# maruchitatsuki/python-based-Sequential-Monte-Carlo-method-with-likelihood-tempering

Hardware: AMD Instinct MI355X
Metric: particle-mutation-steps/sec (higher is better)
Workload: dtype f64

## Files before the change

include/smc_hip.h:

```cpp
#ifndef SMC_HIP_H
#define SMC_HIP_H

#include <stddef.h>
#include <stdint.h>

#ifdef __cplusplus
extern "C" {
#endif

#define SMC_ABI_VERSION 3
#define SMC_MAX_DIM 8
#define SMC_MAX_ESS_CAND 16
#define SMC_MAX_RANKS 64

#define SMC_SET_PRED 0
#define SMC_SET_FILT 1

#define SMC_PRIOR_UNIFORM 0
#define SMC_PRIOR_NORMAL 1
#define SMC_PRIOR_FLAT 2

#define SMC_PRIOR_MODE_MASK 0
#define SMC_PRIOR_MODE_RATIO_MASK 1
#define SMC_PRIOR_MODE_RATIO 2
// ... 125 lines not shown
                             size_t max_staging_bytes, double *mean, double *sd, double *lower, double *upper, int64_t *n_finite,
                             int64_t *n_failed, int64_t *attempts, double *kernel_ms);
int smc_user_pointwise(smc_ctx *ctx, const double *particle, int64_t n, double *ll, int64_t *n_failed, int64_t *attempts);
int smc_user_pointwise_summary(smc_ctx *ctx, int set, size_t max_staging_bytes, int64_t *n, double *max, double *sum_exp, double *mean,
                               double *m2, double *pit, int64_t *n_failed, int64_t *attempts, double *kernel_ms);
int smc_user_sweep_counters(smc_ctx *ctx, int64_t out[4]);
int smc_meth_sweep_counters(smc_ctx *ctx, int64_t out[4]);
int smc_meth_sweep_check(smc_ctx *ctx, int64_t out[5]);
int smc_meth_download_solves(smc_ctx *ctx, double *flows, int32_t *status, int64_t n);
int smc_set_prior(smc_ctx *ctx, const int *kind, const double *a, const double *b, int dim);
int smc_set_prior_mode(smc_ctx *ctx, int mode);

#define SMC_RESAMPLE_RESIDUAL_SYSTEMATIC 0
#define SMC_RESAMPLE_SYSTEMATIC 1
#define SMC_RESAMPLE_MULTINOMIAL 2
int smc_set_early_reject(smc_ctx *ctx, int enable);
int smc_set_stiff_first(smc_ctx *ctx, int enable);
int smc_set_cost_order(smc_ctx *ctx, int enable);
int smc_set_fast_tail(smc_ctx *ctx, int enable);
int smc_set_share_replicates(smc_ctx *ctx, int enable);
int smc_mm_group_replicates(const double *t, const double *S0, int n_ex, int n_t, int *primary, int *partner);
int smc_mm_share_info(smc_ctx *ctx, int *n_solve, int64_t *shared_attempts);
int smc_set_start_reject(smc_ctx *ctx, int enable);
int smc_mm_start_reject_info(smc_ctx *ctx, int64_t *not_started);
double smc_mm_reject_threshold(double lk1, double gamma, double rr, double sigma, int n_ex, int n_t, double pratio, int in_support);
int smc_set_in_phase(smc_ctx *ctx, int enable);
int smc_set_exact_pow(smc_ctx *ctx, int enable);
int smc_set_resampling(smc_ctx *ctx, int scheme);

int smc_upload_particles(smc_ctx *ctx, int set, const double *aos, int64_t n);
int smc_download_particles(smc_ctx *ctx, int set, double *aos, int64_t n);
int smc_upload_lk(smc_ctx *ctx, int set, const double *lk, int64_t n);
int smc_download_lk(smc_ctx *ctx, int set, double *lk, int64_t n);
int smc_download_accept_flags(smc_ctx *ctx, uint8_t *flags, int64_t n);
int smc_download_item_info(smc_ctx *ctx, int32_t *info, int64_t n);
int smc_download_item_sums(smc_ctx *ctx, double *sums, int64_t n);
int smc_commit_filt_to_pred(smc_ctx *ctx);
int smc_sample_prior_device(smc_ctx *ctx, uint64_t seed, int64_t global_offset);

int smc_loglik(smc_ctx *ctx, int set, int64_t *n_failed, int64_t *rk_attempts);
int smc_mm_loglik_host(smc_ctx *ctx, const double *particle, int64_t n, double *lk, double *pred, int64_t *n_failed,
                       int64_t *rk_attempts);

int smc_max_lk_local(smc_ctx *ctx, double *max_lk);
int smc_ess_partials(smc_ctx *ctx, double max_lk, const double *gm, int n_cand, double *sum_w, double *sum_w2);
int smc_max_lk_global(smc_ctx *ctx, double *max_lk);
// ... 93 lines not shown
```

python-based-sequential-monte-carlo-method-with-likelihood-tempering_amd/binding.py:

```python
from __future__ import annotations

import ctypes
import os
import re

_HERE = os.path.dirname(os.path.abspath(__file__))
LIB_PATH = os.environ.get("SMC_HIP_LIB") or os.path.join(_HERE, "libsmc_hip.so")
HEADER_PATH = os.path.join(os.path.dirname(_HERE), "include", "smc_hip.h")

SMC_SET_PRED, SMC_SET_FILT = 0, 1
SMC_USER_METHOD_RK45, SMC_USER_METHOD_BDF = 0, 1
SMC_USER_MAX_OBS = 8
SMC_USER_MAX_INPUTS, SMC_USER_MAX_KNOTS = 8, 4096
SMC_USER_MAX_EVENTS, SMC_USER_MAX_EVENT_VALUES = 256, 8
SMC_USER_MAX_ROOTS, SMC_USER_MAX_ROOT_FIRES = 4, 256
USER_METHODS = {"RK45": SMC_USER_METHOD_RK45, "BDF": SMC_USER_METHOD_BDF}
SMC_PRIOR_UNIFORM, SMC_PRIOR_NORMAL, SMC_PRIOR_FLAT = 0, 1, 2
SMC_PRIOR_MODE_MASK, SMC_PRIOR_MODE_RATIO_MASK, SMC_PRIOR_MODE_RATIO = 0, 1, 2
PRIOR_MODES = {"mask": 0, "ratio_mask": 1, "ratio": 2}
RESAMPLING = {"residual_systematic": 0, "systematic": 1, "multinomial": 2}
SMC_MAX_ESS_CAND = 16
SMC_PRED_MAX_PROBS = 16
SMC_ABI_VERSION = 3
SMC_SWEEP_COUNTER_WORDS = 14
# ... 88 lines not shown
    "smc_user_model_dump_source7": (cint, [ctypes.c_char_p, cint, cint, cint, cint, cint, cint, cint, cint, cint, cint, cint,
                                            ctypes.c_char_p]),
    "smc_user_predict": (cint, [c_ctx, c_dp, i64, c_dp, c_dp, c_i64p, c_i64p]),
    "smc_user_predict_at": (cint, [c_ctx, c_dp, i64, c_dp, c_dp, cint, cint, c_dp, c_i64p, c_i64p]),
    "smc_user_predict_summary": (cint, [c_ctx, cint, c_dp, c_dp, cint, cint, c_dp, cint, cint, u64, i64, ctypes.c_size_t, c_dp, c_dp,
                                         c_dp, c_dp, c_i64p, c_i64p, c_i64p, c_dp]),
    "smc_user_pointwise": (cint, [c_ctx, c_dp, i64, c_dp, c_i64p, c_i64p]),
    "smc_user_pointwise_summary": (cint, [c_ctx, cint, ctypes.c_size_t, c_i64p, c_dp, c_dp, c_dp, c_dp, c_dp, c_i64p, c_i64p, c_dp]),
    "smc_user_sweep_counters": (cint, [c_ctx, c_i64p]),
    "smc_meth_sweep_counters": (cint, [c_ctx, c_i64p]),
    "smc_meth_sweep_check": (cint, [c_ctx, c_i64p]),
    "smc_meth_download_solves": (cint, [c_ctx, c_dp, ctypes.POINTER(ctypes.c_int32), i64]),
    "smc_set_prior": (cint, [c_ctx, c_ip, c_dp, c_dp, cint]),
    "smc_set_prior_mode": (cint, [c_ctx, cint]),
    "smc_set_resampling": (cint, [c_ctx, cint]),
    "smc_set_early_reject": (cint, [c_ctx, cint]),
    "smc_set_stiff_first": (cint, [c_ctx, cint]),
    "smc_set_cost_order": (cint, [c_ctx, cint]),
    "smc_set_fast_tail": (cint, [c_ctx, cint]),
    "smc_set_share_replicates": (cint, [c_ctx, cint]),
    "smc_mm_group_replicates": (cint, [c_dp, c_dp, cint, cint, c_ip, c_ip]),
    "smc_mm_share_info": (cint, [c_ctx, c_ip, c_i64p]),
    "smc_set_start_reject": (cint, [c_ctx, cint]),
    "smc_mm_start_reject_info": (cint, [c_ctx, c_i64p]),
    "smc_mm_reject_threshold": (ctypes.c_double, [ctypes.c_double, ctypes.c_double, ctypes.c_double, ctypes.c_double, cint, cint,
                                                  ctypes.c_double, cint]),
    "smc_set_in_phase": (cint, [c_ctx, cint]),
    "smc_set_exact_pow": (cint, [c_ctx, cint]),
    "smc_exchange_plan": (cint, [cint, cint, i64, c_i64p, c_i64p, c_i64p, c_i64p, c_i64p, c_i64p, c_i64p, c_i64p, c_i64p, c_i64p]),
    "smc_upload_particles": (cint, [c_ctx, cint, c_dp, i64]),
    "smc_download_particles": (cint, [c_ctx, cint, c_dp, i64]),
    "smc_upload_lk": (cint, [c_ctx, cint, c_dp, i64]),
    "smc_download_lk": (cint, [c_ctx, cint, c_dp, i64]),
    "smc_download_accept_flags": (cint, [c_ctx, c_u8p, i64]),
    "smc_download_item_info": (cint, [c_ctx, ctypes.POINTER(ctypes.c_int32), i64]),
    "smc_download_item_sums": (cint, [c_ctx, c_dp, i64]),
    "smc_debug_set_order": (cint, [c_ctx, ctypes.POINTER(ctypes.c_int32), i64, cint]),
    "smc_commit_filt_to_pred": (cint, [c_ctx]),
    "smc_sample_prior_device": (cint, [c_ctx, u64, i64]),
    "smc_loglik": (cint, [c_ctx, cint, c_i64p, c_i64p]),
    "smc_mm_loglik_host": (cint, [c_ctx, c_dp, i64, c_dp, c_dp, c_i64p, c_i64p]),
    "smc_max_lk_local": (cint, [c_ctx, c_dp]),
    "smc_ess_partials": (cint, [c_ctx, f64, c_dp, cint, c_dp, c_dp]),
    "smc_max_lk_global": (cint, [c_ctx, c_dp]),
    "smc_ess_partials_global": (cint, [c_ctx, f64, c_dp, cint, c_dp, c_dp]),
    "smc_ess_search_global": (cint, [c_ctx, c_dp, cint, cint, c_dp, c_dp, c_dp]),
# ... 87 lines not shown
```

python-based-sequential-monte-carlo-method-with-likelihood-tempering_amd/csrc/mm_kernels.hip:

```cpp
#include <hip/hip_runtime.h>

#include <cstdlib>

#include "mh_control.h"
#include "mm_rk45.h"
#include "solve_sched.h"
#include "philox.h"
#include "prior.h"
#include "smc_internal.h"
#include "reject_bound.h"

namespace smc {

constexpr int kInfoAttemptsMask = 0x1fffffff, kInfoCancelled = 1 << 29, kInfoFailed = 1 << 30;
constexpr double kSumCancelled = -1.0;

#ifndef SMC_STIFF_RATIO
#define SMC_STIFF_RATIO 60.0
#endif
constexpr double kStiffRatio = SMC_STIFF_RATIO;
#ifndef SMC_SOLO_RATIO
#define SMC_SOLO_RATIO 1000.0
#endif
constexpr double kSoloRatio = SMC_SOLO_RATIO;
static_assert(kSoloRatio >= kStiffRatio, "the index-ordered pass skips what either list holds by the stiff predicate alone");
__device__ __forceinline__ bool mm_is_stiff(double Vmax, double Km) { return Km > 0.0 && Vmax > kStiffRatio * Km; }
__device__ __forceinline__ bool mm_is_solo(double Vmax, double Km) { return Km > 0.0 && Vmax > kSoloRatio * Km; }
__device__ __forceinline__ void stiff_list_append(const StiffList &sl, int64_t p, double Vmax, double Km) {
    if (mm_is_solo(Vmax, Km)) {
        const unsigned k = atomicAdd(sl.count + 1, 1u);
        if (k < sl.solo_cap) {
            sl.particles[sl.cap - 1 - (int64_t)k] = (int32_t)p;
            return;
        }
    }
    sl.particles[atomicAdd(sl.count, 1u)] = (int32_t)p;
}
constexpr int kCostBuckets = 128, kCostBlocks = 256;
// ... 251 lines not shown
constexpr int kStartLookFrom = SMC_START_LOOK_FROM;
static_assert(kStartLookFrom >= 1, "group 0 is handed out first: it has no finished sibling");

struct SolveArgs {
    const double *theta;
    int64_t stride, n;
    const uint8_t *p0;
    double *sum_r2;
    int *info;
    double *pred;
    unsigned long long *queue;
    const RejectArgs *rej;
    const int32_t *stiff_list;
    const unsigned *stiff_count;
    int64_t stiff_cap;
    unsigned solo_cap;
    int patience;
    int start_look;
    const int32_t *order;
    const unsigned *n_ordered;
    const SortedProposal *sorted;
    const MHControl *ctl;
};

struct ShareArgs {
    const int *groups;
    int n_solve;
};

#ifdef SMC_NO_OWN_SGPR
template <class T> __device__ __forceinline__ T own_sgpr(T v) { return v; }
#else
__device__ __forceinline__ double own_sgpr(double v) {
    double r;
    asm volatile("s_mov_b64 %0, %1" : "=s"(r) : "s"(v));
    return r;
}
template <class T>
__device__ __forceinline__ T *own_sgpr(T *p) {
    T *r;
    asm volatile("s_mov_b64 %0, %1" : "=s"(r) : "s"(p));
    return r;
}
__device__ __forceinline__ int own_sgpr(int v) {
    int r;
    asm volatile("s_mov_b32 %0, %1" : "=s"(r) : "s"(v));
    return r;
}
#endif

__device__ __forceinline__ double mm_loglik_term(double c0, double sum_r2, double s2) { return c0 - sum_r2 / (2.0 * s2); }

__device__ __forceinline__ void publish_item(double *sums, int *infos, int64_t idx, double sum_r2, int info) {
    __hip_atomic_store(reinterpret_cast<unsigned long long *>(sums) + idx, (unsigned long long)__double_as_longlong(sum_r2),
                       __ATOMIC_RELAXED, __HIP_MEMORY_SCOPE_AGENT);
    infos[idx] = info;
}
__device__ __forceinline__ void publish_item(const SolveArgs &a, int64_t idx, double sum_r2, int info) {
    publish_item(a.sum_r2, a.info, idx, sum_r2, info);
}

__device__ __forceinline__ bool mm_certainly_rejected(const MMModel &mm, const SolveArgs &a, int64_t p, int e_self,
                                                      double partial_self, int e_partner = -1, double partial_partner = 0.0) {
    const double sigma = mm.est_sigma ? a.theta[2 * a.stride + p] : mm.sigma_fixed;
    if (!(sigma > 0.0)) return false;
    const double s2 = sigma * sigma;
    const double c0 = (-0.5 * mm.n_t) * log(2.0 * 3.141592653589793 * s2);
    double lk2_bound = 0.0;
    for (int k = 0; k < mm.n_ex; ++k) {
        double S = 0.0;
        if (k == e_self) {
            S = partial_self;
        } else if (k == e_partner) {
            S = partial_partner;
        } else {
            const double v = sibling_sum(a.sum_r2, (int64_t)k * a.n + p);
            if (v < 0.0) return true;
            if (v == v) S = v;
        }
        lk2_bound += mm_loglik_term(c0, S, s2);
    }
    return reject_bound_fails(*a.rej, p, lk2_bound);
}

template <bool WRITE_PRED, bool EXACT, bool FAST, bool SHARE = false>
struct MMOps {
    struct Item {
        MMItem s;
        int64_t out_idx;
        double *pred;
    };
    static constexpr int kPoolWords = smc::kPoolWords;
    const MMModel &mm;
    const SolveArgs &a;
    const double2 *s_tp;
    const double *s_S0;
    long long n;
    int n_ex, n_t;
    const int32_t *list;
    unsigned n_list;
    const int32_t *solo;
    unsigned n_solo;
    double rtol, atol;
    int patience;
    long long n_pos;
    double *pub_sums;
    int *pub_info;
    double *s_sum2;
    const int *s_grp;
    int look;

    __device__ __forceinline__ double *sum2_word() const { return SHARE ? s_sum2 + threadIdx.x : nullptr; }
    __device__ __forceinline__ int partner_distance(const Item &it) const { return SHARE ? it.s.t_off >> kSharePartnerShift : 0; }
    __device__ __forceinline__ double partner_sum(const Item &it) const { return it.s.i_out == 0 ? 0.0 : *sum2_word(); }

    __device__ __forceinline__ int start(long long p, int e, bool from_list, Item &nb) const {
        const bool masked = !a.n_ordered && a.p0 && a.p0[p] == 0;
        return start_values(p, e, from_list, masked, a.theta[p], a.theta[a.stride + p], mm.est_sigma ? a.theta[2 * a.stride + p] : mm.sigma_fixed, nb);
    }
    __device__ __forceinline__ int start_values(long long p, int e, bool from_list, bool masked, double Vmax, double Km, double sigma,
                                                Item &nb) const {
        int d_e = 0;
        const int g_self = e;
        if (SHARE) {
            const int g = e;
            e = s_grp[2 * g];
            const int partner = s_grp[2 * g + 1];
            d_e = partner < 0 ? 0 : partner - e;
        }
        const int n_ex_data = SHARE ? mm.n_ex : n_ex;
        const int64_t out_idx2 = (int64_t)(e + d_e) * a.n + p;
        nb.out_idx = (int64_t)e * a.n + p;
        nb.pred = nullptr;
        if (!from_list && list && !masked && mm_is_stiff(Vmax, Km)) return kStartSkipped;
        if (look != 0 && !from_list && !masked && g_self >= kStartLookFrom) {
            double fin = 0.0;
            bool dead = false;
            const unsigned long long *sums = reinterpret_cast<const unsigned long long *>(pub_sums) + p;
            for (int k = SHARE ? mm.n_ex : n_ex; k > 0; --k, sums += n) {
                const double v = __longlong_as_double((long long)__hip_atomic_load(sums, __ATOMIC_RELAXED, __HIP_MEMORY_SCOPE_AGENT));
                dead = dead || v < 0.0;
                fin += v >= 0.0 ? v : 0.0;
            }
            const double T = *reinterpret_cast<const double *>(sums);
            if (dead || (fin >= T && fin <= 1.7976931348623157e308)) {
                publish_item(a, nb.out_idx, kSumCancelled, 0 | kInfoCancelled);
                if (SHARE && d_e != 0) publish_item(a, out_idx2, kSumCancelled, 0 | kInfoCancelled);
                return kStartDone;
            }
        }
        if (masked || sigma <= 0.0) {
            publish_item(a, nb.out_idx, 0.0, 0);
            if (SHARE && d_e != 0) publish_item(a, out_idx2, 0.0, 0);
            if (WRITE_PRED) {
                double *pp = a.pred + ((size_t)p * n_ex_data + e) * n_t;
                for (int i = 0; i < n_t; ++i) pp[i] = quiet_nan();
                if (SHARE && d_e != 0)
                    for (int i = 0; i < n_t; ++i) pp[d_e * n_t + i] = quiet_nan();
// ... 97 lines not shown
    __device__ __forceinline__ Item broadcast(const Item &it, int src) const {
        Item u;
        u.s.negVmax = lane_value(it.s.negVmax, src);
        u.s.Km = lane_value(it.s.Km, src);
        u.s.S0 = lane_value(it.s.S0, src);
        u.s.t = lane_value(it.s.t, src);
        u.s.y = lane_value(it.s.y, src);
        u.s.f = lane_value(it.s.f, src);
        u.s.h_abs = lane_value(it.s.h_abs, src);
        u.s.min_step = lane_value(it.s.min_step, src);
        u.s.t_bound = lane_value(it.s.t_bound, src);
        u.s.t_next = lane_value(it.s.t_next, src);
        u.s.sum_r2 = lane_value(it.s.sum_r2, src);
        u.s.t_off = __builtin_amdgcn_readlane(it.s.t_off, src);
        u.s.i_out = __builtin_amdgcn_readlane(it.s.i_out, src);
        u.s.attempts = __builtin_amdgcn_readlane(it.s.attempts, src);
        u.s.rejected = __builtin_amdgcn_readlane((int)it.s.rejected, src) != 0;
        u.out_idx = lane_value_ll(it.out_idx, src);
        u.pred = WRITE_PRED ? (double *)lane_value_ll((long long)it.pred, src) : nullptr;
        if (SHARE) *sum2_word() = lane_value(*sum2_word(), src);
        return u;
    }
    __device__ __forceinline__ bool reject_enabled() const { return a.rej != nullptr; }
    __device__ __forceinline__ bool certainly_rejected(const Item &it) const {
        const int e_self = (int)(it.out_idx / a.n);
        if (SHARE) {
            const int d_e = partner_distance(it);
            return mm_certainly_rejected(mm, a, it.out_idx - (int64_t)e_self * a.n, e_self, it.s.sum_r2, d_e != 0 ? e_self + d_e : -1,
                                         partner_sum(it));
        }
        return mm_certainly_rejected(mm, a, it.out_idx - (int64_t)e_self * a.n, e_self, it.s.sum_r2);
    }
    __device__ __forceinline__ void cancel(Item &it) const {
        publish_item(a, it.out_idx, kSumCancelled, it.s.attempts | kInfoCancelled);
        if (SHARE) {
            const int d_e = partner_distance(it);
            if (d_e != 0) publish_item(a, it.out_idx + (int64_t)d_e * a.n, kSumCancelled, it.s.attempts | kInfoCancelled);
        }
    }
};

template <bool WRITE_PRED, bool EXACT, bool FAST, bool SHARE = false>
__device__ __forceinline__ void mm_solve_body(const MMModel &mm, const SolveArgs &a, const ShareArgs *sh = nullptr) {
    extern __shared__ double2 smem_tp[];
    if (a.ctl && __builtin_amdgcn_readfirstlane(a.ctl->stop)) return;
    const int n_ex = mm.n_ex, n_t = mm.n_t;
    double2 *s_tp = smem_tp;
    double *s_S0 = reinterpret_cast<double *>(s_tp + (SHARE ? 2 : 1) * n_ex * (n_t + 1));
    if (SHARE)
        mm_table_fill_shared(s_tp, mm.t, mm.P_obs, n_ex, n_t, threadIdx.x, blockDim.x, sh->groups, sh->n_solve);
    else
        mm_table_fill(s_tp, mm.t, mm.P_obs, n_ex, n_t, threadIdx.x, blockDim.x);
    if (threadIdx.x < n_ex) s_S0[threadIdx.x] = mm.S0[threadIdx.x];
    double *s_sum2 = s_S0 + ((n_ex + 1) & ~1) + (size_t)(kSolveBlock / kWave) * (kPoolWords * kWave);
// ... 363 lines not shown
                         bool start_look = false) {
    const bool share = share_on(ctx);
    MMModel mm = ctx->mm;
    mm.partner_mask = 0;
    SolveArgs a{};
    a.theta = theta;
    a.stride = stride;
    a.n = n;
    a.p0 = p0;
    a.sum_r2 = ctx->d_sum_r2;
    a.info = ctx->d_info;
    a.pred = pred;
    a.queue = ctx->d_queue;
    a.rej = reject ? ctx->d_reject : nullptr;
    a.stiff_list = sl.particles;
    a.stiff_count = sl.count;
    a.stiff_cap = sl.cap;
    a.solo_cap = sl.solo_cap;
    a.patience = patience;
    a.order = order;
    a.n_ordered = cost_ordered ? cost_n_ordered(ctx) : nullptr;
    a.sorted = static_cast<const SortedProposal *>(ctx->d_sorted);
    a.ctl = ctl;
    a.start_look = reject && start_look;
#ifdef SMC_DEBUG_PATIENCE_ENV
    if (const char *e = getenv("SMC_DEBUG_PATIENCE")) a.patience = atoi(e);
#endif
    if (!queue_cleared) (void)hipMemsetAsync(ctx->d_queue, 0, sizeof(unsigned long long), ctx->stream);
    const size_t lds = solve_lds_bytes(mm.n_ex, mm.n_t, share);
    const bool exact = ctx->exact_pow != 0;
    const bool fast = use_fast_tail(ctx, n);
    void (*kern)(MMModel, SolveArgs) =
        pred ? (exact ? mm_solve_kernel<true, true, false> : fast ? mm_solve_kernel<true, false, true> : mm_solve_kernel<true, false, false>)
             : (exact ? mm_solve_kernel<false, true, false> : fast ? mm_solve_kernel<false, false, true> : mm_solve_kernel<false, false, false>);
    void (*kern_share)(MMModel, SolveArgs, ShareArgs) =
        pred ? (exact ? mm_solve_share_kernel<true, true, false> : fast ? mm_solve_share_kernel<true, false, true> : mm_solve_share_kernel<true, false, false>)
             : (exact ? mm_solve_share_kernel<false, true, false> : fast ? mm_solve_share_kernel<false, false, true> : mm_solve_share_kernel<false, false, false>);
    if (lds > 48 * 1024 && !ctx->solve_lds_raised) {
        hipError_t e = hipSuccess;
        for (const void *f : {reinterpret_cast<const void *>(&mm_solve_kernel<true, true, false>), reinterpret_cast<const void *>(&mm_solve_kernel<true, false, false>),
                              reinterpret_cast<const void *>(&mm_solve_kernel<true, false, true>), reinterpret_cast<const void *>(&mm_solve_kernel<false, true, false>),
                              reinterpret_cast<const void *>(&mm_solve_kernel<false, false, false>), reinterpret_cast<const void *>(&mm_solve_kernel<false, false, true>),
                              reinterpret_cast<const void *>(&mm_solve_share_kernel<true, true, false>), reinterpret_cast<const void *>(&mm_solve_share_kernel<true, false, false>),
                              reinterpret_cast<const void *>(&mm_solve_share_kernel<true, false, true>), reinterpret_cast<const void *>(&mm_solve_share_kernel<false, true, false>),
                              reinterpret_cast<const void *>(&mm_solve_share_kernel<false, false, false>), reinterpret_cast<const void *>(&mm_solve_share_kernel<false, false, true>)})
            if (e == hipSuccess) e = hipFuncSetAttribute(f, hipFuncAttributeMaxDynamicSharedMemorySize, 128 * 1024);
        if (e != hipSuccess) {
// ... 86 lines not shown
```

python-based-sequential-monte-carlo-method-with-likelihood-tempering_amd/csrc/smc_api.hip:

```cpp
#include <hip/hip_runtime.h>
#include <rccl/rccl.h>

#include <cmath>
#include <cstddef>
#include <cstdio>
#include <cstdlib>
#include <chrono>
#include <condition_variable>
#include <cstring>
#include <mutex>
#include <new>

#include "exchange_plan.h"
#include "replicate_groups.h"
#include "smc_internal.h"
#include "stage_kernels.h"

using namespace smc;

static thread_local std::string g_err;

#define HIPC(ctx, call)                                                                                   \
    do {                                                                                                  \
        hipError_t e_ = (call);                                                                           \
// ... 133 lines not shown
const char *smc_last_error(const smc_ctx *ctx) { return ctx ? ctx->err.c_str() : g_err.c_str(); }

int smc_create(smc_ctx **out, int device, int64_t n_local, int64_t n_global, int dim) {
    if (!out) return fail(nullptr, "smc_create: out is NULL");
    *out = nullptr;
    if (n_local <= 0 || n_global < n_local) return fail(nullptr, "smc_create: need 0 < n_local <= n_global");
    if (n_global >= (int64_t)1 << 31) return fail(nullptr, "smc_create: n_global must be < 2^31");
    if (dim < 1 || dim > SMC_MAX_DIM) return fail(nullptr, "smc_create: dim out of range");
    int ndev = 0;
    HIPC((smc_ctx *)nullptr, hipGetDeviceCount(&ndev));
    if (device < 0 || device >= ndev) return fail(nullptr, "smc_create: no such HIP device");
    HIPC((smc_ctx *)nullptr, hipSetDevice(device));
    smc_ctx *c = new (std::nothrow) smc_ctx();
    if (!c) return fail(nullptr, "smc_create: out of host memory");
    c->device = device;
    c->dim = dim;
    c->n_local = n_local;
    c->n_global = n_global;
    {
        const char *e = getenv("SMC_SHARE_REPLICATES");
        c->share_env_off = e ? atoi(e) == 0 : false;
        e = getenv("SMC_START_REJECT");
        c->start_reject_env_off = e ? atoi(e) == 0 : false;
    }
#define CK(call)                                   \
    do {                                           \
        hipError_t e_ = (call);                    \
        if (e_ != hipSuccess) {                    \
            g_err = std::string(#call) + ": " + hipGetErrorString(e_); \
            smc_destroy(c);                        \
            return 1;                              \
        }                                          \
    } while (0)
    CK(hipStreamCreateWithFlags(&c->stream, hipStreamNonBlocking));
    const size_t nb = (size_t)n_local * sizeof(double);
    for (int s = 0; s < 2; ++s) {
        CK(hipMalloc(&c->set[s].theta, nb * dim));
        CK(hipMalloc(&c->set[s].lk, nb));
        CK(hipMemsetAsync(c->set[s].theta, 0, nb * dim, c->stream));
        CK(hipMemsetAsync(c->set[s].lk, 0, nb, c->stream));
        c->set[s].stride = n_local;
    }
    CK(hipMalloc(&c->r_ac, (size_t)n_local));
    CK(hipMemsetAsync(c->r_ac, 0, (size_t)n_local, c->stream));
    CK(hipMalloc(&c->d_counters, sizeof(SweepCounters)));
    CK(hipMalloc(&c->d_queue, 2 * sizeof(unsigned long long)));
// ... 331 lines not shown
    c->order_debug_patience = patience;
    return 0;
}
int smc_set_cost_order(smc_ctx *c, int enable) {
    if (!c) return fail(nullptr, "NULL context");
    c->cost_order = enable != 0;
    return 0;
}
int smc_set_fast_tail(smc_ctx *c, int enable) {
    if (!c) return smc_fail(nullptr, "NULL context");
    c->fast_tail = enable != 0;
    return 0;
}
int smc_set_share_replicates(smc_ctx *c, int enable) {
    if (!c) return fail(nullptr, "NULL context");
    c->share_replicates = enable != 0;
    return 0;
}
int smc_set_start_reject(smc_ctx *c, int enable) {
    if (!c) return fail(nullptr, "NULL context");
    c->start_reject = enable != 0;
    return 0;
}
int smc_mm_start_reject_info(smc_ctx *c, int64_t *not_started) {
    if (!c) return fail(nullptr, "NULL context");
    if (not_started) *not_started = c->w_not_started;
    return 0;
}
double smc_mm_reject_threshold(double lk1, double gamma, double rr, double sigma, int n_ex, int n_t, double pratio, int in_support) {
    return mm_reject_threshold(lk1, gamma, rr, sigma, n_ex, n_t, pratio, in_support);
}
int smc_mm_group_replicates(const double *t, const double *S0, int n_ex, int n_t, int *primary, int *partner) {
    if (!t || !S0 || !primary || !partner || n_ex < 1 || n_t < 1) return -1;
    return group_replicates(t, S0, n_ex, n_t, primary, partner);
}
int smc_mm_share_info(smc_ctx *c, int *n_solve, int64_t *shared_attempts) {
    if (!c) return fail(nullptr, "NULL context");
    if (!c->have_model || c->model_kind != 1) return fail(c, "smc_set_model_mm has not been called");
    HIPC(c, hipSetDevice(c->device));
    if (n_solve) *n_solve = solves_per_particle(c);
    if (shared_attempts) {
        unsigned long long v = 0;
        HIPC(c, hipMemcpyAsync(&v, finish_shared_attempts(c), sizeof v, hipMemcpyDeviceToHost, c->stream));
        HIPC(c, hipStreamSynchronize(c->stream));
        *shared_attempts = (int64_t)v;
    }
// ... 1225 lines not shown
```

python-based-sequential-monte-carlo-method-with-likelihood-tempering_amd/csrc/smc_internal.h:

```cpp
#pragma once
#include <hip/hip_runtime.h>
#include <stdint.h>

#include <string>
#include <vector>

#include "../../include/smc_hip.h"
#include "sweep_args.h"

int smc_fail(smc_ctx *ctx, const char *msg);

namespace smc {

constexpr int kWave = 64;
constexpr int kMaxEx = 16;
constexpr int kMaxNt = 256;
constexpr int kScanBlock = 256;
constexpr int kScanItems = 4;
constexpr int kScanTile = kScanBlock * kScanItems;

struct MMModel {
    const double *t;
    const double *P_obs;
    const double *S0;
// ... 188 lines not shown
    int64_t *d_blk_o = nullptr;
    int64_t *d_rs = nullptr, *h_rs = nullptr;
    int rs_pending = 0;
    int64_t n_tiles = 0;
    double *d_sendbuf = nullptr;
    int64_t sendbuf_cap = 0;
    double *d_recvbuf = nullptr;
    int64_t recvbuf_cap = 0;
    double *d_sum_r2 = nullptr;
    int *d_info = nullptr;
    int64_t item_cap = 0;
    uint8_t *d_p0 = nullptr;
    double *d_pratio = nullptr;
    int prior_mode = 0;
    int resampling = 0;
    int early_reject = 1;
    double *d_mn_thr = nullptr;
    double *d_mn_blk = nullptr;
    unsigned long long *d_queue = nullptr;
    unsigned long long *d_finish_rows = nullptr;
    smc::RejectArgs *d_reject = nullptr;
    int start_reject = 1;
    bool start_reject_env_off = false;
    bool start_look_pending = false, start_look_idle = false;
    int64_t w_not_started = 0;
    int32_t *d_stiff_list = nullptr;
    unsigned *d_stiff_count = nullptr;
    int stiff_parity = 0;
    int32_t *d_order = nullptr;
    uint8_t *d_bucket = nullptr;
    unsigned *d_order_hist = nullptr;
    void *d_sorted = nullptr;
    int cost_order = 1;
    int order_debug = 0, order_debug_patience = 0;
    int fast_tail = 1;
    int stiff_first = 1;
    int in_phase = 1;
    int64_t last_sweep_items = 0, last_sweep_long_items = 0, pending_sweep_items = 0;
    int share_replicates = 1;
    bool share_env_off = false;
    int n_solve = 0, partner_mask = 0;
    int groups[2 * smc::kMaxEx]{};
    int *d_groups = nullptr;
    int exact_pow = 0;
    bool solve_lds_raised = false;
    int cu_count = 0, solve_blocks_per_cu = 0, solve_blocks_per_cu_fast = 0;
// ... 58 lines not shown
```

python-based-sequential-monte-carlo-method-with-likelihood-tempering_amd/csrc/solve_sched.h:

```cpp
#pragma once
#ifndef __HIPCC_RTC__
#include <hip/hip_runtime.h>
#endif

#ifndef SMC_CHUNK
#define SMC_CHUNK 128
#endif
#ifndef SMC_REFILL_AT
#define SMC_REFILL_AT 24
#endif
#ifndef SMC_POOL_FREE
#define SMC_POOL_FREE 48
#endif
#ifndef SMC_STIFF_PER_CHUNK
#define SMC_STIFF_PER_CHUNK 16
#endif
#ifdef SMC_ISA_MARKS
#define SMC_ISA_MARK(name) asm volatile("; MARK " name)
#else
#define SMC_ISA_MARK(name)
#endif

namespace smc {

// ... 16 lines not shown
    const int lo = __builtin_amdgcn_readlane(__double2loint(v), src);
    const int hi = __builtin_amdgcn_readlane(__double2hiint(v), src);
    return __hiloint2double(hi, lo);
}
__device__ __forceinline__ long long lane_value_ll(long long v, int src) {
    return (long long)(((unsigned long long)(unsigned)__builtin_amdgcn_readlane((int)((unsigned long long)v >> 32), src) << 32) |
                       (unsigned)__builtin_amdgcn_readlane((int)(unsigned)v, src));
}

template <class Ops>
__device__ __forceinline__ int uniform_attempts_plain(const Ops &ops, typename Ops::Item &u, int budget) {
    int st;
    do {
        SMC_ISA_MARK("uniform_tail_attempt");
        st = ops.attempt(u);
    } while (st == 0 && --budget > 0);
    return st;
}

template <class Ops>
__device__ __forceinline__ void run_item_uniform(Ops &ops, typename Ops::Item &u, bool reject) {
    int st = 0;
    bool cancelled = false;
    for (;;) {
        if (reject && __builtin_amdgcn_readfirstlane((int)ops.certainly_rejected(u))) {
            cancelled = true;
            break;
        }
        st = ops.uniform_attempts(u, kRejectCheckEvery);
        if (st != 0) break;
    }
    if (cancelled)
        ops.cancel(u);
    else
        ops.finish(u, st);
}

template <class Ops>
__device__ __forceinline__ void solve_persistent(Ops &ops, unsigned long long *queue, double *s_pool) {
    using Item = typename Ops::Item;
    constexpr int kWave = kSchedWave;
    const int n_ex = ops.n_ex;
    const long long n_pos = ops.positions();
    const unsigned long long n_blk = (unsigned long long)((n_pos + kWave - 1) / kWave);
    const unsigned n_ex_padded = (unsigned)((n_ex + kExPerChunk - 1) / kExPerChunk) * kExPerChunk;
    const unsigned n_list = ops.n_list;
    const unsigned list_cpe = (n_list + kStiffPerChunk - 1) / kStiffPerChunk;
    const unsigned long long q_list_end = (unsigned long long)list_cpe * n_ex * kChunk;
    const unsigned long long n_items = q_list_end + n_blk * kWave * n_ex_padded;
    const int lane = threadIdx.x & (kWave - 1);

    {
// ... 89 lines not shown
                q_lo += take;
            }
        }
        __builtin_amdgcn_wave_barrier();
        {
            const unsigned long long idle_mask = ~__ballot(live);
            const int n_idle = __popcll(idle_mask);
            if (pool_count > 0 && n_idle > 0) {
                const int k = (int)__builtin_amdgcn_mbcnt_hi((unsigned)(idle_mask >> 32),
                                                             __builtin_amdgcn_mbcnt_lo((unsigned)idle_mask, 0u));
                const int n_take = n_idle < pool_count ? n_idle : pool_count;
                if (!live && k < n_take) {
                    ops.unpack(it, s_pool + ((pool_head + k) & (kWave - 1)));
                    live = true;
                }
                pool_head = (pool_head + n_take) & (kWave - 1);
                pool_count -= n_take;
            }
        }
        __builtin_amdgcn_wave_barrier();
        if (!drained && pool_count == 0 && __ballot(live) == 0ull) continue;
        if (drained && pool_count == 0) {
            const bool reject = ops.reject_enabled();
            for (;;) {
                const unsigned long long tail_mask = __ballot(live);
                const int n_live = __popcll(tail_mask);
                if (n_live == 0) break;
                if (n_live == 1) {
                    const int src = __ffsll((unsigned long long)tail_mask) - 1;
                    Item u = ops.broadcast(it, src);
                    run_item_uniform(ops, u, reject);
                    live = false;
                    break;
                }
                int n_now, since_check = kRejectCheckEvery;
                do {
                    if (live) {
                        if (reject && ++since_check > kRejectCheckEvery) {
                            since_check = 0;
                            if (ops.certainly_rejected(it)) {
                                ops.cancel(it);
                                live = false;
                            }
                        }
                    }
                    if (live) {
                        SMC_ISA_MARK("lane_tail_attempt");
                        const int st = ops.attempt(it);
                        if (st != 0) {
                            ops.finish(it, st);
                            live = false;
                        }
                    }
                    n_now = __popcll(__ballot(live));
                } while (n_now == n_live);
            }
            break;
        }
        const int patience = ops.patience;
        int idle_now, waited = 0;
        do {
            SMC_ISA_MARK("bulk_attempt");
// ... 16 lines not shown
```

python-based-sequential-monte-carlo-method-with-likelihood-tempering_amd/csrc/user_item_ops.h:

```cpp
#ifndef SMC_USER_PRED
#define SMC_USER_PRED 0
#endif
#if SMC_USER_PRED
#define smc_user_item smc_user_item_pred
#define smc_user_solve_kernel smc_user_predict_kernel
#endif
#include "sweep_args.h"
#include "reject_bound.h"
#include "solve_sched.h"
#define NS SMC_USER_NS
#ifdef SMC_USER_ROOTS
#include "user_root.h"
#endif
namespace smc_user_item {
__device__ __forceinline__ double py_min(double a, double b) { return (b < a) ? b : a; }
__device__ __forceinline__ double py_max(double a, double b) { return (b > a) ? b : a; }

#ifdef SMC_USER_NOBS
using DataRec = smc_obs::Rec;
__device__ __forceinline__ double t_bound_of(const DataRec *tp, int n_t) { return tp[n_t].y[0]; }
template <class It>
__device__ __forceinline__ void emit(It &it, const double *yy, const double *theta, const double *cond, double t_out, const double *obs) {
#if defined(SMC_USER_NOISE) && SMC_USER_NOISE
    smc_obs::emit_noise<SMC_USER_PRED, It::kFuseOutputs>(it.sr2, it.pred, it.nz, yy, theta, cond, t_out, obs);
// ... 195 lines not shown
        publish_work(it);
        publish(it.out_idx, -1.0, (int)(it.attempts & 0x1fffffffu) | (1 << 29));
    }
    __device__ __forceinline__ Item broadcast(const Item &it, int src) const {
        Item u;
        Integ::broadcast(u.s, it.s, src);
#pragma unroll
        for (int c = 0; c < SMC_USER_DIM; ++c) u.th[c] = smc::lane_value(it.th[c], src);
#if defined(SMC_USER_NOISE) && SMC_USER_NOISE
#pragma unroll
        for (int k = 0; k < smc_obs::kObs; ++k) {
            u.s.nz.w[k] = smc::lane_value(it.s.nz.w[k], src);
#if SMC_USER_NOISE_PROP
            u.s.nz.q[k] = smc::lane_value(it.s.nz.q[k], src);
#endif
        }
#endif
        u.out_idx = smc::lane_value_ll(it.out_idx, src);
        u.e = __builtin_amdgcn_readlane(it.e, src);
        u.attempts = (unsigned)__builtin_amdgcn_readlane((int)it.attempts, src);
        return u;
    }
    __device__ __forceinline__ bool reject_enabled() const { return a.rej != nullptr; }
#if defined(SMC_USER_NOISE) && SMC_USER_NOISE
    __device__ __forceinline__ bool certainly_rejected(const Item &it) const {
        const long long p = particle(it);
        if (!smc_obs::noise_valid(it.th, a.n_ex, a.n_t)) return false;
        double la[smc_obs::kObs];
#pragma unroll
        for (int k = 0; k < smc_obs::kObs; ++k) la[k] = log(smc_obs::noise_add(it.th, k, a.n_ex, a.n_t) * smc_obs::noise_scale(k, a.n_ex, a.n_t));
        double lk2_bound = 0.0;
        for (int k = 0; k < a.n_ex; ++k) {
            double S = 0.0;
            if (k == it.e) {
                S = it.s.sr2;
            } else {
                const double v = smc::sibling_sum(a.sum_r2, (long long)k * a.n + p);
                if (v < 0.0) return true;
                if (v == v) S = v;
            }
            lk2_bound += smc_obs::noise_floor_of(k, la, a.n_ex, a.n_t) - S;
        }
        return smc::reject_bound_fails(*a.rej, p, lk2_bound);
    }
#else
    __device__ __forceinline__ bool certainly_rejected(const Item &it) const {
// ... 60 lines not shown
```

python-based-sequential-monte-carlo-method-with-likelihood-tempering_amd/driver.py:

```python
from __future__ import annotations

import math
import time
from dataclasses import dataclass, field

import numpy as np

from .binding import SMC_MAX_ESS_CAND, SMC_SET_FILT, SMC_SET_PRED
from .comm import SingleComm


@dataclass
class SMCSettings:
    n_particle: int = 1000
    ess_limit: float = 0.5
    mhstep_factor: float = 0.5
    mhstep_factor_cov: float = 0.5
    ad_mhstep_num: int = 20
    mhstep_num: int = 5
    r_threshold: float = 0.5
    r_threshold_f: float = 0.7
    r_threshold_min: float = 0.1
    d_gamma_max: float = 1
    gm_reduction_itr: int = 80
    gm_reduction_rate: float = 0.7
    itr_max: int = 50
    est_sigma: bool = True
    sigma_true: float = 5
    seed: int = 20250205
    rtol: float = 1e-3
    atol: float = 1e-6
    prior_mode: str = "mask"
    resampling: str = "residual_systematic"
    ess_search: str = "backoff"
    ess_bisect_tol: float = 1e-9
    early_reject: bool = True
    share_replicates: bool = True
    start_reject: bool = True
    stiff_first: bool = True
    in_phase: bool = True
    cost_order: bool = True
    exact_pow: object = None
    defer_resample: bool = True
    pinned_results: bool = True
    mh_batch: object = "auto"
    priors: dict = field(default_factory=lambda: {
        "Vmax": {"dist": "uniform", "low": 0, "high": 10},
        "Km": {"dist": "uniform", "low": 0, "high": 10},
        "sigma": {"dist": "uniform", "low": 0, "high": 10},
    })

    @property
    def num_est_params(self):
        return len(self.priors)

    def w_cov(self):
        d = self.num_est_params
        w = np.ones((d, d))
        for i in range(d):
            w[i, :] = self.mhstep_factor_cov
            w[i, i] = self.mhstep_factor
# ... 232 lines not shown
                         "stream (step << 16) | j would repeat")
    comm = comm or SingleComm()
    n = s.n_particle
    d = s.num_est_params
    world, rank = comm.size, comm.rank
    n_local = engine.n_local
    assert n_local * world == n, "n_particle must equal world * n_local"
    lo = rank * n_local
    w_cov = s.w_cov()
    engine.set_prior_mode(s.prior_mode)
    engine.set_resampling(s.resampling)
    if hasattr(engine, "set_early_reject"):
        engine.set_early_reject(s.early_reject)
    if hasattr(engine, "set_stiff_first"):
        engine.set_stiff_first(s.stiff_first)
    mm_shared0 = None
    if getattr(engine, "model", ("",))[0] == "mm" and hasattr(engine, "set_share_replicates"):
        engine.set_share_replicates(s.share_replicates)
        mm_shared0 = engine.share_info()["rk_attempts_shared"]
    mm_not_started0 = None
    if getattr(engine, "model", ("",))[0] == "mm" and hasattr(engine, "set_start_reject"):
        engine.set_start_reject(s.start_reject)
        mm_not_started0 = engine.start_reject_info()["solves_not_started"]
    if hasattr(engine, "set_in_phase"):
        engine.set_in_phase(s.in_phase)
    if hasattr(engine, "set_cost_order"):
        engine.set_cost_order(s.cost_order)
    if hasattr(engine, "set_exact_pow"):
        engine.set_exact_pow(rng == "numpy" if s.exact_pow is None else bool(s.exact_pow))
    start_time = time.perf_counter()
    stats = {"rk_attempts": 0, "rk_attempts_mh": 0, "n_failed": 0, "mutation_sweeps": 0, "ess_iters": 0,
             "ess_launches": 0, "ess_syncs": 0, "ess_search_s": 0.0, "particle_mutation_steps": 0,
             "mh_syncs": 0, "mh_noop_sweeps": 0}

    meth = getattr(engine, "model", ("",))[0] == "methanation"

    def account(info, counters=None):
        stats["rk_attempts"] += info["rk_attempts"]
        stats["n_failed"] += info["n_failed"]
        if meth:
            if counters is None:
                k8, chk = engine.meth_sweep_counters(), engine.meth_sweep_check()
            else:
                k8 = {"bdf_steps": counters["rk_attempts"], "newton_iters": counters["newton_iters"],
                      "factorisations": counters["factorisations"], "failed_solves": counters["failed_solves"]}
                chk = counters
# ... 186 lines not shown
```

python-based-sequential-monte-carlo-method-with-likelihood-tempering_amd/engine.py:

```python
from __future__ import annotations

import ctypes

import numpy as np

from . import binding as B
from .binding import SMC_SET_FILT, SMC_SET_PRED, SmcError, check, lib


def _dp(a):
    return a.ctypes.data_as(B.c_dp)


def _f64(a, shape=None):
    a = np.ascontiguousarray(a, dtype=np.float64)
    if shape is not None and tuple(a.shape) != tuple(shape):
        raise ValueError(f"expected shape {shape}, got {a.shape}")
    return a


class _PinnedPool:

    def __init__(self, cap_bytes=1 << 30):
        import threading
# ... 312 lines not shown

    def set_fast_tail(self, enable=True):
        if "smc_set_fast_tail" in B.MISSING:
            return
        self._ck(self.L.smc_set_fast_tail(self.ctx, int(bool(enable))), "smc_set_fast_tail")

    def set_share_replicates(self, enable=True):
        if "smc_set_share_replicates" in B.MISSING:
            return
        self._ck(self.L.smc_set_share_replicates(self.ctx, int(bool(enable))), "smc_set_share_replicates")

    def share_info(self):
        if "smc_mm_share_info" in B.MISSING:
            return {"n_solve": self.model[1], "rk_attempts_shared": 0}
        ns, sh = ctypes.c_int(0), ctypes.c_int64(0)
        self._ck(self.L.smc_mm_share_info(self.ctx, ctypes.byref(ns), ctypes.byref(sh)), "smc_mm_share_info")
        return {"n_solve": ns.value, "rk_attempts_shared": sh.value}

    def set_start_reject(self, enable=True):
        if "smc_set_start_reject" in B.MISSING:
            return
        self._ck(self.L.smc_set_start_reject(self.ctx, int(bool(enable))), "smc_set_start_reject")

    def start_reject_info(self):
        if "smc_mm_start_reject_info" in B.MISSING:
            return {"solves_not_started": 0}
        v = ctypes.c_int64(0)
        self._ck(self.L.smc_mm_start_reject_info(self.ctx, ctypes.byref(v)), "smc_mm_start_reject_info")
        return {"solves_not_started": v.value}

    def set_stiff_first(self, enable=True):
        if "smc_set_stiff_first" in B.MISSING:
            return
        self._ck(self.L.smc_set_stiff_first(self.ctx, int(bool(enable))), "smc_set_stiff_first")

    def set_resampling(self, scheme):
        k = B.RESAMPLING[scheme] if isinstance(scheme, str) else int(scheme)
        self._ck(self.L.smc_set_resampling(self.ctx, k), "smc_set_resampling")

    def upload_particles(self, which, aos):
        aos = _f64(aos)
        assert aos.ndim == 2 and aos.shape[1] == self.dim
        self._ck(self.L.smc_upload_particles(self.ctx, which, _dp(aos), aos.shape[0]), "smc_upload_particles")

    def download_particles(self, which, n=None, pinned=False):
        n = self.n_local if n is None else n
# ... 427 lines not shown
```

Before: 490.4 million.

## Publish boxed partial residual sums so sibling solves can reject earlier

In-progress solves now publish their running residual sum, stored as a float packed into a NaN payload, to the shared sums array. Sibling rejection checks unbox these partial sums to tighten the certain-reject bound, and use a direct threshold comparison when the start threshold is present. This is meant to cancel doomed ODE solves sooner. The check cadence also changes to a separate constant, which adds more atomic stores and more frequent checks per item.

```diff
diff --git a/include/smc_hip.h b/include/smc_hip.h
--- a/include/smc_hip.h
+++ b/include/smc_hip.h
@@ -171,6 +171,7 @@
 int smc_mm_group_replicates(const double *t, const double *S0, int n_ex, int n_t, int *primary, int *partner);
 int smc_mm_share_info(smc_ctx *ctx, int *n_solve, int64_t *shared_attempts);
 int smc_set_start_reject(smc_ctx *ctx, int enable);
+int smc_set_partial_sums(smc_ctx *ctx, int enable);
 int smc_mm_start_reject_info(smc_ctx *ctx, int64_t *not_started);
 double smc_mm_reject_threshold(double lk1, double gamma, double rr, double sigma, int n_ex, int n_t, double pratio, int in_support);
 int smc_set_in_phase(smc_ctx *ctx, int enable);
diff --git a/python-based-sequential-monte-carlo-method-with-likelihood-tempering_amd/binding.py b/python-based-sequential-monte-carlo-method-with-likelihood-tempering_amd/binding.py
--- a/python-based-sequential-monte-carlo-method-with-likelihood-tempering_amd/binding.py
+++ b/python-based-sequential-monte-carlo-method-with-likelihood-tempering_amd/binding.py
@@ -134,6 +134,7 @@
     "smc_mm_group_replicates": (cint, [c_dp, c_dp, cint, cint, c_ip, c_ip]),
     "smc_mm_share_info": (cint, [c_ctx, c_ip, c_i64p]),
     "smc_set_start_reject": (cint, [c_ctx, cint]),
+    "smc_set_partial_sums": (cint, [c_ctx, cint]),
     "smc_mm_start_reject_info": (cint, [c_ctx, c_i64p]),
     "smc_mm_reject_threshold": (ctypes.c_double, [ctypes.c_double, ctypes.c_double, ctypes.c_double, ctypes.c_double, cint, cint,
                                                   ctypes.c_double, cint]),
diff --git a/python-based-sequential-monte-carlo-method-with-likelihood-tempering_amd/csrc/mm_kernels.hip b/python-based-sequential-monte-carlo-method-with-likelihood-tempering_amd/csrc/mm_kernels.hip
--- a/python-based-sequential-monte-carlo-method-with-likelihood-tempering_amd/csrc/mm_kernels.hip
+++ b/python-based-sequential-monte-carlo-method-with-likelihood-tempering_amd/csrc/mm_kernels.hip
@@ -9,11 +9,17 @@
 #include "prior.h"
 #include "smc_internal.h"
 #include "reject_bound.h"
+#include "partial_sum_box.h"
 
 namespace smc {
 
 constexpr int kInfoAttemptsMask = 0x1fffffff, kInfoCancelled = 1 << 29, kInfoFailed = 1 << 30;
 constexpr double kSumCancelled = -1.0;
+#ifndef SMC_PARTIAL_LOOK_EVERY
+#define SMC_PARTIAL_LOOK_EVERY 128
+#endif
+constexpr int kPartialLookEvery = SMC_PARTIAL_LOOK_EVERY;
+static_assert(kPartialLookEvery >= 1 && kPartialLookEvery <= kRejectCheckEvery, "more looks than the scheduler's own cadence, not fewer");
 
 #ifndef SMC_STIFF_RATIO
 #define SMC_STIFF_RATIO 60.0
@@ -311,6 +317,7 @@
     const SortedProposal *sorted;
     const MHControl *ctl;
 };
+constexpr int kLookNone = 0, kLookThreshold = 1, kLookThresholdPartial = 2, kLookPartial = -1;
 
 struct ShareArgs {
     const int *groups;
@@ -350,7 +357,7 @@
 }
 
 __device__ __forceinline__ bool mm_certainly_rejected(const MMModel &mm, const SolveArgs &a, int64_t p, int e_self,
-                                                      double partial_self, int e_partner = -1, double partial_partner = 0.0) {
+                                                      double partial_self, int e_partner, double partial_partner, bool unbox) {
     const double sigma = mm.est_sigma ? a.theta[2 * a.stride + p] : mm.sigma_fixed;
     if (!(sigma > 0.0)) return false;
     const double s2 = sigma * sigma;
@@ -366,6 +373,7 @@
             const double v = sibling_sum(a.sum_r2, (int64_t)k * a.n + p);
             if (v < 0.0) return true;
             if (v == v) S = v;
+            else if (unbox) S = unbox_partial(v);
         }
         lk2_bound += mm_loglik_term(c0, S, s2);
     }
@@ -398,6 +406,8 @@
     double *s_sum2;
     const int *s_grp;
     int look;
+    __device__ __forceinline__ bool look_threshold() const { return look > 0; }
+    __device__ __forceinline__ bool look_partial() const { return (look & 2) != 0; }
 
     __device__ __forceinline__ double *sum2_word() const { return SHARE ? s_sum2 + threadIdx.x : nullptr; }
     __device__ __forceinline__ int partner_distance(const Item &it) const { return SHARE ? it.s.t_off >> kSharePartnerShift : 0; }
@@ -422,7 +432,7 @@
         nb.out_idx = (int64_t)e * a.n + p;
         nb.pred = nullptr;
         if (!from_list && list && !masked && mm_is_stiff(Vmax, Km)) return kStartSkipped;
-        if (look != 0 && !from_list && !masked && g_self >= kStartLookFrom) {
+        if (look_threshold() && !from_list && !masked && g_self >= kStartLookFrom) {
             double fin = 0.0;
             bool dead = false;
             const unsigned long long *sums = reinterpret_cast<const unsigned long long *>(pub_sums) + p;
@@ -566,14 +576,46 @@
         return u;
     }
     __device__ __forceinline__ bool reject_enabled() const { return a.rej != nullptr; }
+    __device__ __forceinline__ int look_every(bool reject) const { return reject && look_partial() ? kPartialLookEvery : kRejectCheckEvery; }
+    __device__ __forceinline__ void publish_partial(const Item &it) const {
+        if (!look_partial()) return;
+        unsigned long long *slot = reinterpret_cast<unsigned long long *>(pub_sums) + it.out_idx;
+        __hip_atomic_store(slot, (unsigned long long)__double_as_longlong(box_partial(it.s.sum_r2)), __ATOMIC_RELAXED, __HIP_MEMORY_SCOPE_AGENT);
+        if (SHARE) {
+            const int d_e = partner_distance(it);
+            if (d_e != 0)
+                __hip_atomic_store(slot + (int64_t)d_e * n, (unsigned long long)__double_as_longlong(box_partial(partner_sum(it))),
+                                   __ATOMIC_RELAXED, __HIP_MEMORY_SCOPE_AGENT);
+        }
+    }
+    __device__ __forceinline__ int threshold_reached(const Item &it, int e_self, int e_partner) const {
+        const int64_t p = it.out_idx - (int64_t)e_self * n;
+        const int n_data = SHARE ? mm.n_ex : n_ex;
+        double fin = it.s.sum_r2 + (e_partner >= 0 ? partner_sum(it) : 0.0);
+        bool dead = false;
+        for (int k = 0; k < n_data; ++k) {
+            if (k == e_self || k == e_partner) continue;
+            const double v = sibling_sum(pub_sums, (int64_t)k * n + p);
+            dead = dead || v < 0.0;
+            fin += v >= 0.0 ? v : unbox_partial(v);
+        }
+        const double T = pub_sums[(int64_t)n_data * n + p];
+        if (dead || (fin >= T && fin <= 1.7976931348623157e308)) return 1;
+        return T <= 1.7976931348623157e308 ? 0 : -1;
+    }
     __device__ __forceinline__ bool certainly_rejected(const Item &it) const {
         const int e_self = (int)(it.out_idx / a.n);
+        int e_partner = -1;
         if (SHARE) {
             const int d_e = partner_distance(it);
-            return mm_certainly_rejected(mm, a, it.out_idx - (int64_t)e_self * a.n, e_self, it.s.sum_r2, d_e != 0 ? e_self + d_e : -1,
-                                         partner_sum(it));
-        }
-        return mm_certainly_rejected(mm, a, it.out_idx - (int64_t)e_self * a.n, e_self, it.s.sum_r2);
+            if (d_e != 0) e_partner = e_self + d_e;
+        }
+        if (look_partial() && look_threshold()) {
+            const int reached = threshold_reached(it, e_self, e_partner);
+            if (reached >= 0) return reached != 0;
+        }
+        return mm_certainly_rejected(mm, a, it.out_idx - (int64_t)e_self * a.n, e_self, it.s.sum_r2, e_partner,
+                                     e_partner >= 0 ? partner_sum(it) : 0.0, look_partial());
     }
     __device__ __forceinline__ void cancel(Item &it) const {
         publish_item(a, it.out_idx, kSumCancelled, it.s.attempts | kInfoCancelled);
@@ -983,7 +1025,8 @@
     a.n_ordered = cost_ordered ? cost_n_ordered(ctx) : nullptr;
     a.sorted = static_cast<const SortedProposal *>(ctx->d_sorted);
     a.ctl = ctl;
-    a.start_look = reject && start_look;
+    const bool partial = reject && ctx->partial_sums != 0 && !ctx->partial_sums_env_off;
+    a.start_look = reject && start_look ? (partial ? kLookThresholdPartial : kLookThreshold) : (partial ? kLookPartial : kLookNone);
 #ifdef SMC_DEBUG_PATIENCE_ENV
     if (const char *e = getenv("SMC_DEBUG_PATIENCE")) a.patience = atoi(e);
 #endif
diff --git a/python-based-sequential-monte-carlo-method-with-likelihood-tempering_amd/csrc/partial_sum_box.h b/python-based-sequential-monte-carlo-method-with-likelihood-tempering_amd/csrc/partial_sum_box.h
--- /dev/null
+++ b/python-based-sequential-monte-carlo-method-with-likelihood-tempering_amd/csrc/partial_sum_box.h
@@ -0,0 +1,43 @@
+#pragma once
+#include <stdint.h>
+#include <string.h>
+
+#ifndef __HIPCC__
+#ifndef __host__
+#define __host__
+#define __device__
+#endif
+#endif
+
+namespace smc {
+
+__host__ __device__ inline uint64_t partial_bits_of(double v) {
+    uint64_t b;
+    memcpy(&b, &v, sizeof b);
+    return b;
+}
+__host__ __device__ inline double partial_double_of(uint64_t b) {
+    double v;
+    memcpy(&v, &b, sizeof v);
+    return v;
+}
+
+__host__ __device__ inline uint32_t partial_float_bits(double s) {
+    const uint64_t b = partial_bits_of(s);
+    constexpr uint64_t kFltMin = 0x3810000000000000ULL;
+    constexpr uint64_t kFltMax = 0x47efffffe0000000ULL;
+    constexpr uint64_t kInf = 0x7ff0000000000000ULL;
+    if (b < kFltMin || b > kInf) return 0u;
+    if (b >= kFltMax) return 0x7f7fffffu;
+    return (uint32_t)((b >> 29) - ((uint64_t)(1023 - 127) << 23));
+}
+
+__host__ __device__ inline double box_partial(double s) { return partial_double_of(0x7ff8000000000000ULL | partial_float_bits(s)); }
+
+__host__ __device__ inline double unbox_partial(double v) {
+    const uint32_t f = (uint32_t)partial_bits_of(v);
+    if (f < 0x00800000u || f > 0x7f7fffffu) return 0.0;
+    return partial_double_of(((uint64_t)f << 29) + ((uint64_t)(1023 - 127) << 52));
+}
+
+}
diff --git a/python-based-sequential-monte-carlo-method-with-likelihood-tempering_amd/csrc/smc_api.hip b/python-based-sequential-monte-carlo-method-with-likelihood-tempering_amd/csrc/smc_api.hip
--- a/python-based-sequential-monte-carlo-method-with-likelihood-tempering_amd/csrc/smc_api.hip
+++ b/python-based-sequential-monte-carlo-method-with-likelihood-tempering_amd/csrc/smc_api.hip
@@ -179,6 +179,8 @@
         c->share_env_off = e ? atoi(e) == 0 : false;
         e = getenv("SMC_START_REJECT");
         c->start_reject_env_off = e ? atoi(e) == 0 : false;
+        e = getenv("SMC_PARTIAL_SUMS");
+        c->partial_sums_env_off = e ? atoi(e) == 0 : false;
     }
 #define CK(call)                                   \
     do {                                           \
@@ -556,6 +558,11 @@
     c->start_reject = enable != 0;
     return 0;
 }
+int smc_set_partial_sums(smc_ctx *c, int enable) {
+    if (!c) return fail(nullptr, "NULL context");
+    c->partial_sums = enable != 0;
+    return 0;
+}
 int smc_mm_start_reject_info(smc_ctx *c, int64_t *not_started) {
     if (!c) return fail(nullptr, "NULL context");
     if (not_started) *not_started = c->w_not_started;
diff --git a/python-based-sequential-monte-carlo-method-with-likelihood-tempering_amd/csrc/smc_internal.h b/python-based-sequential-monte-carlo-method-with-likelihood-tempering_amd/csrc/smc_internal.h
--- a/python-based-sequential-monte-carlo-method-with-likelihood-tempering_amd/csrc/smc_internal.h
+++ b/python-based-sequential-monte-carlo-method-with-likelihood-tempering_amd/csrc/smc_internal.h
@@ -234,6 +234,8 @@
     smc::RejectArgs *d_reject = nullptr;
     int start_reject = 1;
     bool start_reject_env_off = false;
+    int partial_sums = 1;
+    bool partial_sums_env_off = false;
     bool start_look_pending = false, start_look_idle = false;
     int64_t w_not_started = 0;
     int32_t *d_stiff_list = nullptr;
diff --git a/python-based-sequential-monte-carlo-method-with-likelihood-tempering_amd/csrc/solve_sched.h b/python-based-sequential-monte-carlo-method-with-likelihood-tempering_amd/csrc/solve_sched.h
--- a/python-based-sequential-monte-carlo-method-with-likelihood-tempering_amd/csrc/solve_sched.h
+++ b/python-based-sequential-monte-carlo-method-with-likelihood-tempering_amd/csrc/solve_sched.h
@@ -62,12 +62,14 @@
 __device__ __forceinline__ void run_item_uniform(Ops &ops, typename Ops::Item &u, bool reject) {
     int st = 0;
     bool cancelled = false;
+    const int every = ops.look_every(reject);
     for (;;) {
+        if (reject) ops.publish_partial(u);
         if (reject && __builtin_amdgcn_readfirstlane((int)ops.certainly_rejected(u))) {
             cancelled = true;
             break;
         }
-        st = ops.uniform_attempts(u, kRejectCheckEvery);
+        st = ops.uniform_attempts(u, every);
         if (st != 0) break;
     }
     if (cancelled)
@@ -203,6 +205,7 @@
         if (!drained && pool_count == 0 && __ballot(live) == 0ull) continue;
         if (drained && pool_count == 0) {
             const bool reject = ops.reject_enabled();
+            const int every = ops.look_every(reject);
             for (;;) {
                 const unsigned long long tail_mask = __ballot(live);
                 const int n_live = __popcll(tail_mask);
@@ -214,11 +217,12 @@
                     live = false;
                     break;
                 }
-                int n_now, since_check = kRejectCheckEvery;
+                int n_now, since_check = every;
                 do {
                     if (live) {
-                        if (reject && ++since_check > kRejectCheckEvery) {
+                        if (reject && ++since_check > every) {
                             since_check = 0;
+                            ops.publish_partial(it);
                             if (ops.certainly_rejected(it)) {
                                 ops.cancel(it);
                                 live = false;
diff --git a/python-based-sequential-monte-carlo-method-with-likelihood-tempering_amd/csrc/user_item_ops.h b/python-based-sequential-monte-carlo-method-with-likelihood-tempering_amd/csrc/user_item_ops.h
--- a/python-based-sequential-monte-carlo-method-with-likelihood-tempering_amd/csrc/user_item_ops.h
+++ b/python-based-sequential-monte-carlo-method-with-likelihood-tempering_amd/csrc/user_item_ops.h
@@ -241,6 +241,8 @@
         return u;
     }
     __device__ __forceinline__ bool reject_enabled() const { return a.rej != nullptr; }
+    __device__ __forceinline__ int look_every(bool) const { return smc::kRejectCheckEvery; }
+    __device__ __forceinline__ void publish_partial(const Item &) const {}
 #if defined(SMC_USER_NOISE) && SMC_USER_NOISE
     __device__ __forceinline__ bool certainly_rejected(const Item &it) const {
         const long long p = particle(it);
diff --git a/python-based-sequential-monte-carlo-method-with-likelihood-tempering_amd/driver.py b/python-based-sequential-monte-carlo-method-with-likelihood-tempering_amd/driver.py
--- a/python-based-sequential-monte-carlo-method-with-likelihood-tempering_amd/driver.py
+++ b/python-based-sequential-monte-carlo-method-with-likelihood-tempering_amd/driver.py
@@ -37,6 +37,7 @@
     early_reject: bool = True
     share_replicates: bool = True
     start_reject: bool = True
+    partial_sums: bool = True
     stiff_first: bool = True
     in_phase: bool = True
     cost_order: bool = True
@@ -315,6 +316,8 @@
     if getattr(engine, "model", ("",))[0] == "mm" and hasattr(engine, "set_start_reject"):
         engine.set_start_reject(s.start_reject)
         mm_not_started0 = engine.start_reject_info()["solves_not_started"]
+    if getattr(engine, "model", ("",))[0] == "mm" and hasattr(engine, "set_partial_sums"):
+        engine.set_partial_sums(s.partial_sums)
     if hasattr(engine, "set_in_phase"):
         engine.set_in_phase(s.in_phase)
     if hasattr(engine, "set_cost_order"):
diff --git a/python-based-sequential-monte-carlo-method-with-likelihood-tempering_amd/engine.py b/python-based-sequential-monte-carlo-method-with-likelihood-tempering_amd/engine.py
--- a/python-based-sequential-monte-carlo-method-with-likelihood-tempering_amd/engine.py
+++ b/python-based-sequential-monte-carlo-method-with-likelihood-tempering_amd/engine.py
@@ -358,6 +358,11 @@
             return
         self._ck(self.L.smc_set_start_reject(self.ctx, int(bool(enable))), "smc_set_start_reject")
 
+    def set_partial_sums(self, enable=True):
+        if "smc_set_partial_sums" in B.MISSING:
+            return
+        self._ck(self.L.smc_set_partial_sums(self.ctx, int(bool(enable))), "smc_set_partial_sums")
+
     def start_reject_info(self):
         if "smc_mm_start_reject_info" in B.MISSING:
             return {"solves_not_started": 0}
```

Measured after the change: 486.7 million. Within noise of the previous version (-0.8%).
